# slbouknight/accelerated-ray-tracer

Hardware: AMD Instinct MI355X
Metric: Mrays/s, 1200x800 random scene @ 500 spp (frame ms in ms_per_step) (higher is better)
Workload: dtype f32

## Files before the change

accelerated-ray-tracer_amd/csrc/rt_abi.hip:

```cpp
#include <hip/hip_runtime.h>

#include <algorithm>
#include <cfloat>
#include <utility>
#include <cmath>
#include <functional>
#include <cstdio>
#include <cstring>
#include <string>
#include <vector>

#include "../../include/rt_abi.h"
#include "rt_call_buffers.h"
#include "rt_device.h"
#include "rt_frame_plan.h"
#include "rt_handoff_order.h"
#include "rt_refit_host.h"
#include "rt_scene_plan.h"

namespace {

struct device_info {
    bool ready = false;
    int num_cu = 256;
// ... 1553 lines not shown
    *count_out = (int64_t)count;
    const size_t n = count < (size_t)cap ? count : (size_t)cap;
    if (n == 0) return RT_OK;
    HIPCHK(hipMemcpy(entries, s->d_handoff, n * sizeof(unsigned long long), hipMemcpyDeviceToHost));
    HIPCHK(hipMemcpy(served, s->plan.tail_ordered ? s->d_handoff_ordered : s->d_handoff, n * sizeof(unsigned long long), hipMemcpyDeviceToHost));
    std::vector<rt_pixel_state> h_state(s->pixel_capacity);
    HIPCHK(hipMemcpy(h_state.data(), s->d_state, h_state.size() * sizeof(rt_pixel_state), hipMemcpyDeviceToHost));
    for (size_t i = 0; i < n; ++i) {
        const uint32_t pix = (uint32_t)entries[i];
        costs[i] = pix < h_state.size() ? h_state[pix].cost : 0u;
    }
    return RT_OK;
}

enum { ORDER_SEAM_SLACK = 3 };
rt_status rt_debug_order_handoff(const unsigned long long* entries, const uint32_t* costs, int64_t n, int32_t sample_begin, int32_t sample_end,
                                 int32_t tail_waves, unsigned long long* out, uint32_t* overrun_out) {
    if (!overrun_out) return invalid("rt_debug_order_handoff: null argument");
    if (n < 0 || n > (1ll << 24) || (n > 0 && (!entries || !costs || !out))) return invalid("rt_debug_order_handoff: n must be 0 .. 2^24 and the arrays non-null");
    if (sample_begin < 0 || sample_end < sample_begin) return invalid("rt_debug_order_handoff: bad sample range");
    if (tail_waves < 1 || tail_waves > (1 << 20)) return invalid("rt_debug_order_handoff: tail_waves must be 1 .. 2^20");
    for (int64_t i = 0; i < n; ++i)
        if ((int64_t)(uint32_t)entries[i] >= n) return invalid("rt_debug_order_handoff: an entry's pixel is not below n");
    RT_TRY(use_device(g_device));
    call_memory mem;
    rt_handoff_order_params hp;
    memset(&hp, 0, sizeof(hp));
    const size_t most = (size_t)RT_HANDOFF_ORDER_MAX_PER_WAVE * (size_t)tail_waves;
    hp.cap = (uint32_t)n; hp.min_items = (uint32_t)(RT_HANDOFF_ORDER_MIN_PER_WAVE * tail_waves); hp.max_items = (uint32_t)(most < (size_t)n ? most : (size_t)n);
    hp.cost_begin = sample_begin; hp.sample_end = sample_end;
    unsigned long long *d_queue = nullptr, *d_ordered = nullptr;
    rt_pixel_state* d_state = nullptr;
    unsigned int* d_pushed = nullptr;
    const size_t scratch_bytes = rt_handoff_order_scratch_words(hp.max_items) * sizeof(unsigned int);
    HIPCHK(mem.get((void**)&d_queue, (size_t)(n + ORDER_SEAM_SLACK) * sizeof(unsigned long long)));
    HIPCHK(mem.get((void**)&d_ordered, (size_t)(n + ORDER_SEAM_SLACK) * sizeof(unsigned long long)));
    HIPCHK(mem.get((void**)&d_state, (size_t)(n + 1) * sizeof(rt_pixel_state)));
    HIPCHK(mem.get((void**)&d_pushed, sizeof(unsigned int)));
    HIPCHK(mem.get((void**)&hp.scratch, scratch_bytes));
    std::vector<rt_pixel_state> h_state((size_t)n + 1);
    for (int64_t i = 0; i < n; ++i) h_state[(size_t)i].cost = costs[i];
    const unsigned int h_pushed = (unsigned int)n + ORDER_SEAM_SLACK;
    HIPCHK(hipMemset(d_queue, 0, (size_t)(n + ORDER_SEAM_SLACK) * sizeof(unsigned long long)));
    if (n > 0) HIPCHK(hipMemcpy(d_queue, entries, (size_t)n * sizeof(unsigned long long), hipMemcpyHostToDevice));
    HIPCHK(hipMemcpy(d_state, h_state.data(), h_state.size() * sizeof(rt_pixel_state), hipMemcpyHostToDevice));
    HIPCHK(hipMemset(d_ordered, 0xFF, (size_t)(n + ORDER_SEAM_SLACK) * sizeof(unsigned long long)));
    HIPCHK(hipMemcpy(d_pushed, &h_pushed, sizeof(h_pushed), hipMemcpyHostToDevice));
    HIPCHK(hipMemset(hp.scratch, 0, scratch_bytes));
    hp.queue = d_queue; hp.ordered = d_ordered; hp.state = d_state; hp.pushed = d_pushed;
    HIPCHK(rt_launch_handoff_order(hp, nullptr));
    HIPCHK(hipDeviceSynchronize());
    if (n > 0) HIPCHK(hipMemcpy(out, d_ordered, (size_t)n * sizeof(unsigned long long), hipMemcpyDeviceToHost));
    unsigned long long spare[ORDER_SEAM_SLACK];
    HIPCHK(hipMemcpy(spare, d_ordered + n, sizeof(spare), hipMemcpyDeviceToHost));
    *overrun_out = 0u;
    for (const unsigned long long w : spare) *overrun_out += w != ~0ull ? 1u : 0u;
    return RT_OK;
}

rt_status rt_debug_counters(rt_scene* s, unsigned long long* out16) {
    if (!s || !out16) return invalid("null argument");
    RT_TRY(use_device(s->device));
    HIPCHK(hipMemcpy(out16, s->d_ray_counter + 1, 16 * sizeof(unsigned long long), hipMemcpyDeviceToHost));
    return RT_OK;
}
rt_status rt_debug_stage_cycles(rt_scene* s, unsigned long long* out10) {
    if (!s || !out10) return invalid("null argument");
    RT_TRY(use_device(s->device));
    HIPCHK(hipMemcpy(out10, s->d_ray_counter + 17, 10 * sizeof(unsigned long long), hipMemcpyDeviceToHost));
    return RT_OK;
}
rt_status rt_debug_wave_ends(rt_scene* s, unsigned long long* out, int n) {
    if (!s || !out || n < 0 || n > 2 * RT_DIAG_BINS) return invalid("bad argument");
    RT_TRY(use_device(s->device));
    HIPCHK(hipMemcpy(out, s->d_ray_counter + RT_DIAG_HIST_SLOT, (size_t)n * sizeof(unsigned long long), hipMemcpyDeviceToHost));
    return RT_OK;
}
rt_status rt_debug_wave_last(rt_scene* s, unsigned long long* out, int n_waves) {
    if (!s || !out || n_waves < 0 || n_waves > RT_DIAG_MAX_WAVES) return invalid("bad argument");
    RT_TRY(use_device(s->device));
    HIPCHK(hipMemcpy(out, s->d_ray_counter + RT_DIAG_WAVE_SLOT, (size_t)2 * n_waves * sizeof(unsigned long long), hipMemcpyDeviceToHost));
    return RT_OK;
}

namespace {
enum { RANK_PARAM_WORDS = 20, RANK_INFO_WORDS = 13 };
static_assert(sizeof(rt_rank_info) == RANK_INFO_WORDS * 4, "rt_debug_rank / rt_debug_rank_info copy rt_rank_info as 13 words");
}

rt_status rt_debug_rank(const uint32_t* cost, const uint32_t* tile_cost, uint64_t rays, const uint32_t* params, uint32_t* tile_order,
                        uint32_t* cost_out, uint32_t* heavy_pixels, uint32_t* info13) {
    if (!cost || !tile_cost || !params || !tile_order || !cost_out || !heavy_pixels || !info13) return invalid("rt_debug_rank: null argument");
    rt_rank_params rp;
    memset(&rp, 0, sizeof(rp));
    const int32_t* ip = reinterpret_cast<const int32_t*>(params);
    rp.n_pixels = params[0]; rp.n_tiles = params[1]; rp.heavy_cap = params[2];
    rp.max_grid = params[3]; rp.waves_per_wg = params[4]; rp.normal_need = params[5];
    rp.sparse_stride = ip[6]; rp.semi_stride = ip[7]; rp.sparse_percent = ip[8]; rp.sparse_work_percent = ip[9];
    rp.tier_possible = ip[10]; rp.tier1_pixels = ip[11]; rp.tier1_depth = ip[12]; rp.tier_wgs_cap = ip[13];
    rp.tier_waves_per_main_wg = ip[14]; rp.nx = ip[15]; rp.smooth_percent = ip[16];
    memcpy(&rp.heavy_factor, params + 17, 4); memcpy(&rp.sparse_factor, params + 18, 4); memcpy(&rp.tier1_factor, params + 19, 4);
    if (rp.n_pixels < 1u || rp.n_pixels >= (1u << 31)) return invalid("rt_debug_rank: n_pixels must be 1 .. 2^31 - 1");
    if (rp.n_tiles < 1u || rp.n_tiles > rp.n_pixels) return invalid("rt_debug_rank: n_tiles must be 1 .. n_pixels");
    if (rp.heavy_cap < 1u || rp.heavy_cap > (1u << 24)) return invalid("rt_debug_rank: heavy_cap must be 1 .. 2^24");
    if (rp.max_grid > (1u << 20) || rp.normal_need > (1u << 20)) return invalid("rt_debug_rank: max_grid and normal_need must be at most 2^20");
    if (rp.waves_per_wg < 1u || rp.waves_per_wg > 16u) return invalid("rt_debug_rank: waves_per_wg must be 1 .. 16");
    if (rp.sparse_stride < 0 || rp.sparse_stride > 64 || rp.semi_stride < 0 || rp.semi_stride > 64) return invalid("rt_debug_rank: sparse_stride and semi_stride must be 0 .. 64");
    if (rp.sparse_percent < 0 || rp.sparse_percent > 100 || rp.sparse_work_percent < 0 || rp.sparse_work_percent > 100 || rp.smooth_percent < 0 || rp.smooth_percent > 100)
        return invalid("rt_debug_rank: sparse_percent, sparse_work_percent and smooth_percent must be 0 .. 100");
    if (rp.tier1_pixels < 0 || rp.tier1_depth < 0 || rp.tier1_depth > 65536 || rp.tier_wgs_cap < 0 || rp.tier_waves_per_main_wg < 0)
        return invalid("rt_debug_rank: tier1_pixels, tier1_depth (at most 65536), tier_wgs_cap and tier_waves_per_main_wg must not be negative");
    if (rp.nx < 1 || (uint32_t)rp.nx > rp.n_pixels) return invalid("rt_debug_rank: nx must be 1 .. n_pixels");
    float top = 0.f;
    for (const float fac : {rp.heavy_factor, rp.sparse_factor, rp.tier1_factor}) {
        if (!(fac >= 0.f) || !(fac <= 1000.f)) return invalid("rt_debug_rank: the three factors must be 0 .. 1000");
        top = fac > top ? fac : top;
    }
    if (!((double)rays / (double)rp.n_pixels * (double)top + 1.0 < 4294967296.0)) return invalid("rt_debug_rank: rays / n_pixels x the largest factor must stay below 2^32");
    RT_TRY(use_device(g_device));
    call_memory mem;
    unsigned int *d_tile_cost = nullptr, *d_tile_order = nullptr;
    unsigned long long* d_rays = nullptr;
    HIPCHK(mem.get((void**)&rp.state, (size_t)rp.n_pixels * sizeof(rt_pixel_state)));
    HIPCHK(mem.get((void**)&d_tile_cost, (size_t)rp.n_tiles * sizeof(unsigned int)));
    HIPCHK(mem.get((void**)&d_tile_order, (size_t)rp.n_tiles * sizeof(unsigned int)));
    HIPCHK(mem.get((void**)&d_rays, sizeof(unsigned long long)));
    HIPCHK(mem.get((void**)&rp.heavy_list, (size_t)rp.heavy_cap * sizeof(unsigned long long)));
    HIPCHK(mem.get((void**)&rp.heavy_pixels, (size_t)rp.heavy_cap * sizeof(unsigned int)));
    HIPCHK(mem.get((void**)&rp.info, sizeof(rt_rank_info)));
    rp.tile_cost = d_tile_cost; rp.tile_order = d_tile_order; rp.ray_counter = d_rays;
    std::vector<rt_pixel_state> h_state(rp.n_pixels);
    for (uint32_t i = 0; i < rp.n_pixels; ++i) h_state[i].cost = cost[i];
    const unsigned long long h_rays = rays;
    HIPCHK(hipMemcpy(rp.state, h_state.data(), (size_t)rp.n_pixels * sizeof(rt_pixel_state), hipMemcpyHostToDevice));
    HIPCHK(hipMemcpy(d_tile_cost, tile_cost, (size_t)rp.n_tiles * sizeof(unsigned int), hipMemcpyHostToDevice));
    HIPCHK(hipMemcpy(d_rays, &h_rays, sizeof(h_rays), hipMemcpyHostToDevice));
    HIPCHK(hipMemset(d_tile_order, 0xFF, (size_t)rp.n_tiles * sizeof(unsigned int)));
    HIPCHK(hipMemset(rp.heavy_list, 0xFF, (size_t)rp.heavy_cap * sizeof(unsigned long long)));
    HIPCHK(hipMemset(rp.heavy_pixels, 0xFF, (size_t)rp.heavy_cap * sizeof(unsigned int)));
    HIPCHK(hipMemset(rp.info, 0xFF, sizeof(rt_rank_info)));
    HIPCHK(rt_launch_rank(rp, nullptr));
    HIPCHK(hipDeviceSynchronize());
    HIPCHK(hipMemcpy(h_state.data(), rp.state, (size_t)rp.n_pixels * sizeof(rt_pixel_state), hipMemcpyDeviceToHost));
    for (uint32_t i = 0; i < rp.n_pixels; ++i) cost_out[i] = h_state[i].cost;
    HIPCHK(hipMemcpy(tile_order, d_tile_order, (size_t)rp.n_tiles * sizeof(unsigned int), hipMemcpyDeviceToHost));
    HIPCHK(hipMemcpy(heavy_pixels, rp.heavy_pixels, (size_t)rp.heavy_cap * sizeof(unsigned int), hipMemcpyDeviceToHost));
    HIPCHK(hipMemcpy(info13, rp.info, sizeof(rt_rank_info), hipMemcpyDeviceToHost));
    return RT_OK;
}

rt_status rt_debug_prior(const uint32_t* cal_cost, int32_t cal_nx, int32_t cal_ny, int32_t nx, int32_t ny, int32_t tile_rows, int32_t tile_first,
                         int32_t tile_stride, uint32_t* cost_out, uint32_t* tile_cost_out, uint64_t* total_out) {
    if (!cal_cost || !cost_out || !tile_cost_out || !total_out) return invalid("rt_debug_prior: null argument");
    if (cal_nx < 1 || cal_ny < 1 || (long long)cal_nx * cal_ny >= (1ll << 31)) return invalid("rt_debug_prior: bad calibration grid size");
    rt_frame_desc f;
    memset(&f, 0, sizeof(f));
    f.nx = nx; f.ny = ny; f.tile_rows = tile_rows; f.tile_first = tile_first; f.tile_stride = tile_stride;
    frame_geometry g;
    RT_TRY(check_frame("rt_debug_prior", &f, false, STATE_FRAME_TEXTS, g));
    if (g.local_rows == 0) return invalid("rt_debug_prior: the partition has no rows");
    RT_TRY(use_device(g_device));
    rt_prior_params pp;
    memset(&pp, 0, sizeof(pp));
    pp.cal_nx = cal_nx; pp.cal_ny = cal_ny; pp.nx = nx; pp.ny = ny; pp.local_rows = g.local_rows; pp.tiles_x = g.tiles_x;
    pp.tile_rows = tile_rows; pp.tile_first = tile_first; pp.tile_stride = tile_stride;
    const size_t n_pixels = g.n_pixels, n_tiles = (size_t)g.tiles_x * (size_t)g.tiles_y, n_cal = (size_t)cal_nx * (size_t)cal_ny;
// ... 702 lines not shown
```

accelerated-ray-tracer_amd/csrc/rt_device.h:

```cpp
#pragma once
#include <hip/hip_runtime.h>
#include <stdint.h>

#include "../../include/rt_abi.h"

#define RT_PERSISTENT_THREADS 512
#ifndef RT_LEAN_MIN_WAVES
#define RT_LEAN_MIN_WAVES 4
#endif
#ifndef RT_LEAN_MAX_THREADS
#define RT_LEAN_MAX_THREADS 512
#endif
#define RT_HEAVY_MAX_THREADS 768
#define RT_HEAVY_MIN_WAVES 3

#define RT_TIER_THREADS 256
enum { RT_DIAG_BINS = 192, RT_DIAG_T0_SLOT = 32, RT_DIAG_HIST_SLOT = 33, RT_DIAG_WAVE_SLOT = 33 + 2 * 192 + 7, RT_DIAG_MAX_WAVES = 8192,
       RT_COUNTER_BYTES = (33 + 2 * 192 + 7 + 2 * 8192) * 8 };
enum { RT_KERNEL_PIXEL = 0, RT_KERNEL_STAGED = 3 };

struct rt_pixel_state {
    uint32_t rng[6];
    float col[3];
    uint32_t cost;
};

struct rt_rank_info {
    uint32_t heavy_items;
    uint32_t heavy_threshold;
    uint32_t tier1_items;
    uint32_t tier2_items;
    int32_t tier1_wgs;
    int32_t main_skip_wgs;
    int32_t sparse_wgs;
    int32_t sparse_stride;
    int32_t semi_wgs;
    int32_t semi_stride;
    uint32_t threshold1;
    uint32_t threshold2;
    uint32_t collected;
};

struct rt_rank_params {
    rt_pixel_state* state;
    const unsigned int* tile_cost;
    unsigned int* tile_order;
    const unsigned long long* ray_counter;
    unsigned long long* heavy_list;
    unsigned int* heavy_pixels;
    rt_rank_info* info;
    uint32_t n_pixels, n_tiles, heavy_cap;
    uint32_t max_grid, waves_per_wg, normal_need;
    int32_t sparse_stride;
    int32_t semi_stride;
    int32_t sparse_percent;
    int32_t sparse_work_percent;
    int32_t tier_possible;
    int32_t tier1_pixels;
    int32_t tier1_depth;
    int32_t tier_wgs_cap;
    int32_t tier_waves_per_main_wg;
    int32_t nx, smooth_percent;
    float heavy_factor, sparse_factor, tier1_factor;
};

#define RT_NODE_SKIP(stored) (~(stored))
#define RT_WALK_PRIM_TABLE_BYTES(n_nodes) ((4 * (n_nodes) + 15) & ~15)

struct rt_scene_dev {
    const rt_node* nodes;
    const rt_node* nodes_ref;
    const rt_sphere* spheres;
    const rt_quad* quads;
    const rt_box* boxes;
    const rt_instance* instances;
    const rt_medium* media;
    const rt_material* materials;
    const rt_texture* textures;
    const uint8_t* images;
    int32_t n_nodes, n_nodes_ref, n_spheres, n_materials, n_textures;
    float bound[3];
    float bound_pad;
    const float4* leaf_lo;
    const float4* leaf_hi;
    const float* slot_ranges;
    int32_t n_leaves, n_slots;
    int32_t n_media_leaves;
    int32_t media_ord[2];
    rt_camera camera;
};

enum { RT_WC_DEAD = 64,
       RT_WC_PUSHED = 65,
       RT_WC_TAIL_HEAD = 66,
       RT_WORK_COUNTER_BYTES = 512 };
struct rt_frame_params {
    float* fb;
    unsigned long long* ray_counter;
    unsigned int* work_counter;
    unsigned int* pixel_cost;
    unsigned int* node_pass;
// ... 359 lines not shown
```

accelerated-ray-tracer_amd/csrc/rt_kernel_tier.h:

```cpp
#pragma once
#include "rt_device_funcs.h"
#include "rt_launch.h"

struct TierView {
    const float4* lo;
    const float4* hi;
    const float* ranges;
    int n_slots;
    int n_media;
    int med_ord0, med_ord1;
};

template <bool FEW>
DEV float wave_min_of(float v, bool have) {
    if (!FEW) {
        float r = have ? v : FLT_MAX;
#pragma unroll
        for (int off = 32; off > 0; off >>= 1) r = fminf(r, __shfl_xor(r, off, 64));
        return r;
    }
    unsigned long long m = __ballot(have);
    float r = FLT_MAX;
    while (m != 0ull) {
        const int l = __ffsll((long long)m) - 1;
        m &= m - 1ull;
        r = fminf(r, __int_as_float(__builtin_amdgcn_readlane(__float_as_int(v), l)));
    }
    return r;
}

template <bool SPHERES_ONLY>
DEV bool trace_wave(const TierView& tv, const SceneView& sc, const Ray& r, HitInfo& best) {
    const f3 inv = mk3(1.0f / r.d.x, 1.0f / r.d.y, 1.0f / r.d.z);
    const float tmin = 0.001f;
    const float a = dot(r.d, r.d);
    const int lane = (int)(threadIdx.x & 63u);
    const bool finite = inv_is_finite(inv);
    bool meets = false;
    if (finite && lane < tv.n_slots) {
        const float* q = tv.ranges + lane * 8;
        float t_enter, t_exit;
        slab_interval(make_float4(q[0], q[1], q[2], 0.f), make_float4(q[3], q[4], q[5], 0.f), r.o, inv, tmin, t_enter, t_exit);
        meets = !(t_exit <= t_enter);
    }
    unsigned long long slot_mask = __ballot(meets);
    float bt = FLT_MAX;
    int bord = -1;
    int32_t bleaf = -1, binst = -1;
    bool bincl = false, anomaly = false;
    float pre0 = FLT_MAX, pre1 = FLT_MAX;
    if (SPHERES_ONLY) {
        int np = 0;
        int32_t p0 = -1, p1 = -1;
        int o0 = 0, o1 = 0;
        float e0 = 0.f, e1 = 0.f;
        auto sphere_candidate = [&](int32_t prim, int ord, float t_enter) {
            float t;
            if (sphere_test_a(sc.spheres[RT_PRIM_INDEX(prim)], r, a, tmin, FLT_MAX, t)) {
                if (!(t > t_enter)) anomaly = true;
                if (t < bt || (t == bt && ord < bord)) { bt = t; bord = ord; bleaf = prim; }
            }
        };
        auto note = [&](bool pass, int32_t prim, int ord, float t_enter) {
            const bool overflow = pass && np >= 2;
            if (pass && np == 0) { p0 = prim; o0 = ord; e0 = t_enter; }
            if (pass && np == 1) { p1 = prim; o1 = ord; e1 = t_enter; }
            if (pass) ++np;
            if (__ballot(overflow) != 0ull) { if (overflow) sphere_candidate(prim, ord, t_enter); }
        };
        while (slot_mask != 0ull) {
            const int k0 = __ffsll((long long)slot_mask) - 1;
            slot_mask &= slot_mask - 1ull;
            const bool two = slot_mask != 0ull;
            const int k1 = two ? __ffsll((long long)slot_mask) - 1 : k0;
            if (two) slot_mask &= slot_mask - 1ull;
            const int ord0 = k0 * 64 + lane, ord1 = k1 * 64 + lane;
            const float4 lo0 = tv.lo[ord0], hi0 = tv.hi[ord0], lo1 = tv.lo[ord1], hi1 = tv.hi[ord1];
            float t_enter, t_exit;
            slab_interval(lo0, hi0, r.o, inv, tmin, t_enter, t_exit);
            note(__float_as_int(lo0.w) >= 0 && !(t_exit <= t_enter), __float_as_int(lo0.w), ord0, t_enter);
            if (two) {
                slab_interval(lo1, hi1, r.o, inv, tmin, t_enter, t_exit);
                note(__float_as_int(lo1.w) >= 0 && !(t_exit <= t_enter), __float_as_int(lo1.w), ord1, t_enter);
            }
        }
        if (__ballot(np >= 1) != 0ull) { if (np >= 1) sphere_candidate(p0, o0, e0); }
        if (__ballot(np >= 2) != 0ull) { if (np >= 2) sphere_candidate(p1, o1, e1); }
    } else {
    auto candidate = [&](int32_t prim, int32_t inst1, int ord8, float t_enter) {
        Ray q = r;
        if (inst1 != 0) q = to_object_space(sc.instances[inst1 - 1], r);
        float t;
        const bool is_quad = RT_PRIM_KIND(prim) == RT_PRIM_QUAD;
        const bool hit = is_quad ? quad_test(sc.quads[RT_PRIM_INDEX(prim)], q, tmin, FLT_MAX, t) : sphere_test(sc.spheres[RT_PRIM_INDEX(prim)], q, tmin, FLT_MAX, t);
        if (hit) {
            if (!(t > t_enter)) anomaly = true;
            const bool better = t < bt || (t == bt && (is_quad ? (!bincl || ord8 > bord) : (!bincl && ord8 < bord)));
            if (better) { bt = t; bord = ord8; bleaf = prim; binst = inst1 - 1; bincl = is_quad; }
            if ((ord8 >> 3) < tv.med_ord0) pre0 = fminf(pre0, t);
            if ((ord8 >> 3) < tv.med_ord1) pre1 = fminf(pre1, t);
        }
    };
    while (slot_mask != 0ull) {
        const int k = __ffsll((long long)slot_mask) - 1;
        slot_mask &= slot_mask - 1ull;
        const int ord = k * 64 + lane;
        const float4 lo4 = tv.lo[ord], hi4 = tv.hi[ord];
        const int32_t prim = __float_as_int(lo4.w), xw = __float_as_int(hi4.w);
        float t_enter, t_exit;
        slab_interval(lo4, hi4, r.o, inv, tmin, t_enter, t_exit);
        const bool pass = prim >= 0 && !(t_exit <= t_enter) && RT_PRIM_KIND(prim) != RT_PRIM_MEDIUM;
        const bool six = (xw & (1 << 30)) != 0;
        const unsigned long long m1 = __ballot(pass && !six), m6 = __ballot(pass && six);
        if (m1 != 0ull) { if (pass && !six) candidate(prim, xw & 0x3FFFFFFF, ord * 8, t_enter); }
        if (m6 != 0ull) {
            const int need = 6 * __popcll(m6);
            for (int base = 0; base < need; base += 64) {
                const int j = base + lane;
                const int T = j / 6, f = j - 6 * T;
                int lo_l = 0, hi_l = 63;
#pragma unroll
                for (int it = 0; it < 6; ++it) {
                    const int mid = (lo_l + hi_l) >> 1;
                    const bool enough = __popcll(m6 & ((2ull << mid) - 1ull)) > T;
                    hi_l = enough ? mid : hi_l;
                    lo_l = enough ? lo_l : mid + 1;
                }
                const int src = lo_l & 63;
                const int32_t p0 = __shfl(prim, src, 64), x0 = __shfl(xw, src, 64);
                const float te = __shfl(t_enter, src, 64);
                if (j < need) candidate(p0 + f, x0 & 0x3FFFFFFF, (k * 64 + src) * 8 + f, te);
            }
        }
    }
    }
    if (!finite || __ballot(anomaly) != 0ull) return trace<SPHERES_ONLY>(sc, r, best);
    float tm[2] = {FLT_MAX, FLT_MAX};
    bool hm[2] = {false, false};
    if (!SPHERES_ONLY) {
        for (int m = 0; m < tv.n_media; ++m) {
            const int ord = m == 0 ? tv.med_ord0 : tv.med_ord1;
            float limit = wave_min_of<false>(m == 0 ? pre0 : pre1, (m == 0 ? pre0 : pre1) < FLT_MAX);
            if (m == 1 && hm[0]) limit = fminf(limit, tm[0]);
            const float4 lo4 = tv.lo[ord], hi4 = tv.hi[ord];
            const int32_t prim = __builtin_amdgcn_readfirstlane(__float_as_int(lo4.w));
            float t_enter, t_exit;
            slab_interval(lo4, hi4, r.o, inv, tmin, t_enter, t_exit);
            if (!(fminf(t_exit, limit) <= t_enter)) {
                const rt_medium med = uniform_load(sc.media + RT_PRIM_INDEX(prim));
                float t;
                if (medium_test<true>(sc, med, r, tmin, limit, t)) { tm[m] = t; hm[m] = true; }
            }
        }
    }
    const float ts = wave_min_of<SPHERES_ONLY>(bt, bord >= 0);
    const float tmin_all = fminf(ts, fminf(tm[0], tm[1]));
    best.inst = -1;
    if (!(tmin_all < FLT_MAX)) { best.t = FLT_MAX; best.prim = -1; return false; }
    unsigned long long tie = __ballot(bord >= 0 && bt == tmin_all);
    int w_ord = -1, w_lane = -1;
    bool w_incl = false;
    while (tie != 0ull) {
        const int l = __ffsll((long long)tie) - 1;
        tie &= tie - 1ull;
        const int o = __builtin_amdgcn_readlane(bord, l);
        const bool ic = __builtin_amdgcn_readlane(bincl ? 1 : 0, l) != 0;
        const bool take = w_ord < 0 || (ic ? (!w_incl || o > w_ord) : (!w_incl && o < w_ord));
        if (take) { w_ord = o; w_lane = l; w_incl = ic; }
    }
    int w_medium = -1;
    if (!SPHERES_ONLY) {
        for (int m = 0; m < tv.n_media; ++m) {
            if (!hm[m] || tm[m] != tmin_all) continue;
            const int o = (m == 0 ? tv.med_ord0 : tv.med_ord1) * 8;
            if (w_ord < 0 || !w_incl || o > w_ord) { w_ord = o; w_incl = true; w_medium = m; w_lane = -1; }
        }
    }
    best.t = tmin_all;
    if (w_medium >= 0) {
        const float4 lo4 = tv.lo[SPHERES_ONLY ? w_ord : (w_ord >> 3)];
        best.prim = __builtin_amdgcn_readfirstlane(__float_as_int(lo4.w));
        return true;
    }
    best.prim = __builtin_amdgcn_readlane(bleaf, w_lane);
    best.inst = SPHERES_ONLY ? -1 : __builtin_amdgcn_readlane(binst, w_lane);
    return true;
}

template <bool SPHERES_ONLY, int TEX, bool NEED_UV, bool LDS_SCENE>
__global__ void __launch_bounds__(RT_TIER_THREADS, (SPHERES_ONLY && TEX < 2) ? 4 : 3) rt_tier_kernel(rt_scene_dev sd, rt_frame_params fp) {
    extern __shared__ __attribute__((aligned(16))) unsigned char lds[];
    const bool tail = (fp.tail_mode & 1) != 0;
    const rt_rank_info* q = fp.rank;
    const uint32_t n_items = tail ? (fp.work_counter[RT_WC_PUSHED] < fp.handoff_cap ? fp.work_counter[RT_WC_PUSHED] : fp.handoff_cap) : q->tier1_items;
    const int my_wgs = tail ? (int)((n_items + RT_TIER_THREADS / 64 - 1) / (RT_TIER_THREADS / 64)) : q->tier1_wgs;
    if ((int)blockIdx.x >= my_wgs) return;
    if (fp.tier_priority >= 3) __builtin_amdgcn_s_setprio(3);
    else if (fp.tier_priority == 2) __builtin_amdgcn_s_setprio(2);
    else if (fp.tier_priority == 1) __builtin_amdgcn_s_setprio(1);

    SceneView sc;
    sc.nodes = sd.nodes; sc.spheres = sd.spheres; sc.quads = sd.quads; sc.boxes = sd.boxes; sc.instances = sd.instances;
    sc.media = sd.media; sc.materials = sd.materials; sc.textures = sd.textures; sc.images = sd.images; sc.n_nodes = sd.n_nodes;
    TierView tv;
    {
        const int n_pad = sd.n_slots * 64;
        float4* dlo = reinterpret_cast<float4*>(lds);
        float4* dhi = dlo + n_pad;
        float4* dr = dhi + n_pad;
        for (int k = (int)threadIdx.x; k < n_pad; k += (int)blockDim.x) { dlo[k] = sd.leaf_lo[k]; dhi[k] = sd.leaf_hi[k]; }
        const float4* sr = reinterpret_cast<const float4*>(sd.slot_ranges);
        for (int k = (int)threadIdx.x; k < sd.n_slots * 2; k += (int)blockDim.x) dr[k] = sr[k];
        if (LDS_SCENE) {
            float4* dsph = dr + sd.n_slots * 2;
            const float4* s4 = reinterpret_cast<const float4*>(sd.spheres);
            for (int k = (int)threadIdx.x; k < sd.n_spheres * 2; k += (int)blockDim.x) dsph[k] = s4[k];
            sc.spheres = reinterpret_cast<const rt_sphere*>(dsph);
            float4* dmat = dsph + sd.n_spheres * 2;
            const float4* m4 = reinterpret_cast<const float4*>(sd.materials);
            for (int k = (int)threadIdx.x; k < sd.n_materials * 2; k += (int)blockDim.x) dmat[k] = m4[k];
            sc.materials = reinterpret_cast<const rt_material*>(dmat);
            float4* dtex = dmat + sd.n_materials * 2;
            const float4* t4 = reinterpret_cast<const float4*>(sd.textures);
            for (int k = (int)threadIdx.x; k < sd.n_textures * 4; k += (int)blockDim.x) dtex[k] = t4[k];
            sc.textures = reinterpret_cast<const rt_texture*>(dtex);
        }
        __syncthreads();
        tv.lo = dlo; tv.hi = dhi; tv.ranges = reinterpret_cast<const float*>(dr); tv.n_slots = sd.n_slots;
        tv.n_media = SPHERES_ONLY ? 0 : sd.n_media_leaves;
        tv.med_ord0 = tv.n_media > 0 ? sd.media_ord[0] : 0x7FFFFFFF;
        tv.med_ord1 = tv.n_media > 1 ? sd.media_ord[1] : 0x7FFFFFFF;
    }

    unsigned int rays = 0;
#ifdef RT_DIAG
    unsigned long long diag_trace = 0, diag_shade = 0, diag_rays = 0;
    const unsigned long long diag_t0 = __builtin_readcyclecounter();
#endif
    for (;;) {
        uint32_t idx = 0;
        if ((threadIdx.x & 63) == 0) idx = atomicAdd(fp.work_counter + (tail ? RT_WC_TAIL_HEAD : 2), 1u);
        idx = (uint32_t)__builtin_amdgcn_readfirstlane((int)idx);
        if (idx >= n_items) break;
        const unsigned long long item = tail ? fp.handoff_queue[idx] : (unsigned long long)fp.heavy_pixels[idx];
        const uint32_t pix = (uint32_t)item;
        const int first_sample = tail ? (int)(item >> 32) : fp.sample_begin;
        if (tail && (threadIdx.x & 63) == 0) {
            atomicAdd(fp.ray_counter + 28, 1ull); atomicAdd(fp.ray_counter + 29, (unsigned long long)(fp.sample_end - first_sample));
        }
        const int lrow = (int)(pix / (uint32_t)fp.nx), i = (int)(pix - (uint32_t)lrow * (uint32_t)fp.nx);
        const int j = local_to_global_row(fp, lrow);
        rt_xorwow pg;
        f3 pcol;
        uint32_t cost_before;
        {
            const rt_pixel_state st = tail ? fp.handoff_state[pix] : fp.state_in[pix];
            if (fp.fresh && !tail) {
                rt_xorwow_seed(pg, fp.seed_base + (uint64_t)(j * fp.nx + i));
                pcol = mk3(0, 0, 0);
                cost_before = st.cost & 0x80000000u;
            } else {
                pg.v0 = st.rng[0]; pg.v1 = st.rng[1]; pg.v2 = st.rng[2]; pg.v3 = st.rng[3]; pg.v4 = st.rng[4]; pg.d = st.rng[5];
                pcol = mk3(st.col[0], st.col[1], st.col[2]);
                cost_before = st.cost;
            }
        }
        unsigned int pixel_rays = 0;
        for (int sidx = first_sample; sidx < fp.sample_end; ++sidx) {
            const float u = ((float)i + rt_xorwow_uniform(pg)) / (float)fp.nx;
            const float v = ((float)j + rt_xorwow_uniform(pg)) / (float)fp.ny;
            Ray r = camera_get_ray(sd.camera, u, v, pg);
            f3 thr = mk3(1, 1, 1), rad = mk3(0, 0, 0);
            for (int depth = 0; depth < 50; ++depth) {
                HitInfo h;
                ++pixel_rays;
#ifdef RT_DIAG
                const unsigned long long dg0 = __builtin_readcyclecounter();
#endif
                const bool hit_something = trace_wave<SPHERES_ONLY>(tv, sc, r, h);
#ifdef RT_DIAG
                const unsigned long long dg1 = __builtin_readcyclecounter();
                diag_trace += dg1 - dg0; ++diag_rays;
#endif
                if (!hit_something) { rad = fma3(thr, miss_color(fp, r), rad); break; }
                const HitRec rec = resolve_hit<SPHERES_ONLY, NEED_UV>(sc, r, h);
                f3 emitted, attenuation;
                Ray scattered;
                const bool go_on = shade<TEX>(sc, r, rec, pg, emitted, attenuation, scattered);
#ifdef RT_DIAG
                diag_shade += __builtin_readcyclecounter() - dg1;
#endif
                rad = fma3(thr, emitted, rad);
                if (!go_on) break;
                thr = thr * attenuation;
                r = scattered;
            }
            pcol = pcol + rad;
        }
        if ((threadIdx.x & 63) == 0) {
            if (fp.state_out) {
                rt_pixel_state so;
                so.rng[0] = pg.v0; so.rng[1] = pg.v1; so.rng[2] = pg.v2; so.rng[3] = pg.v3; so.rng[4] = pg.v4; so.rng[5] = pg.d;
                so.col[0] = pcol.x; so.col[1] = pcol.y; so.col[2] = pcol.z;
                so.cost = cost_before + pixel_rays;
                fp.state_out[pix] = so;
                if (fp.tile_cost) atomicAdd(&fp.tile_cost[(lrow >> 3) * fp.tiles_x + (i >> 3)], pixel_rays);
            } else {
                store_sum(fp, i, lrow, pcol);
                if (fp.cost_out) fp.cost_out[pix] = (cost_before + pixel_rays) & 0x7FFFFFFFu;
            }
            rays += pixel_rays;
        }
    }
    if ((threadIdx.x & 63) == 0 && rays) atomicAdd(fp.ray_counter, (unsigned long long)rays);
#ifdef RT_DIAG
    if (threadIdx.x == 0 && diag_rays) {
        atomicAdd(fp.ray_counter + 15, diag_trace); atomicAdd(fp.ray_counter + 16, diag_rays);
        atomicAdd(fp.ray_counter + 25, diag_shade); atomicAdd(fp.ray_counter + 26, (unsigned long long)(__builtin_readcyclecounter() - diag_t0));
    }
#endif
}

template <bool SO, int TX, bool UV, bool LS>
static hipError_t rt_launch_tier_variant(const rt_scene_dev& sd, const rt_frame_params& fp, dim3 grid, size_t lds, hipStream_t st) {
    return rt_launch_kernel(rt_tier_kernel<SO, TX, UV, LS>, dim3(RT_TIER_THREADS), grid, lds, st, sd, fp);
}
template <bool SO, int TX, bool UV>
static hipError_t rt_launch_tier_one(const rt_scene_dev& sd, const rt_frame_params& fp, dim3 grid, size_t lds, hipStream_t st) {
    return fp.tier_lds_scene ? rt_launch_tier_variant<SO, TX, UV, true>(sd, fp, grid, lds, st) : rt_launch_tier_variant<SO, TX, UV, false>(sd, fp, grid, lds, st);
}
```

Baseline: 15620.

## Add lean wave-uniform sphere trace, resolve and shade path for tier kernel

```diff
diff --git a/accelerated-ray-tracer_amd/csrc/rt_abi.hip b/accelerated-ray-tracer_amd/csrc/rt_abi.hip
--- a/accelerated-ray-tracer_amd/csrc/rt_abi.hip
+++ b/accelerated-ray-tracer_amd/csrc/rt_abi.hip
@@ -1659,6 +1659,12 @@
     HIPCHK(hipMemcpy(out, s->d_ray_counter + RT_DIAG_WAVE_SLOT, (size_t)2 * n_waves * sizeof(unsigned long long), hipMemcpyDeviceToHost));
     return RT_OK;
 }
+rt_status rt_debug_tier_phases(rt_scene* s, unsigned long long* out, int n) {
+    if (!s || !out || n < 0 || n > 2 * RT_DIAG_TIER_WORDS) return invalid("bad argument");
+    RT_TRY(use_device(s->device));
+    HIPCHK(hipMemcpy(out, s->d_ray_counter + RT_DIAG_TIER_SLOT, (size_t)n * sizeof(unsigned long long), hipMemcpyDeviceToHost));
+    return RT_OK;
+}
 
 namespace {
 enum { RANK_PARAM_WORDS = 20, RANK_INFO_WORDS = 13 };
diff --git a/accelerated-ray-tracer_amd/csrc/rt_device.h b/accelerated-ray-tracer_amd/csrc/rt_device.h
--- a/accelerated-ray-tracer_amd/csrc/rt_device.h
+++ b/accelerated-ray-tracer_amd/csrc/rt_device.h
@@ -16,7 +16,8 @@
 
 #define RT_TIER_THREADS 256
 enum { RT_DIAG_BINS = 192, RT_DIAG_T0_SLOT = 32, RT_DIAG_HIST_SLOT = 33, RT_DIAG_WAVE_SLOT = 33 + 2 * 192 + 7, RT_DIAG_MAX_WAVES = 8192,
-       RT_COUNTER_BYTES = (33 + 2 * 192 + 7 + 2 * 8192) * 8 };
+       RT_DIAG_TIER_SLOT = 33 + 2 * 192 + 7 + 2 * 8192, RT_DIAG_TIER_WORDS = 64,
+       RT_COUNTER_BYTES = (33 + 2 * 192 + 7 + 2 * 8192 + 2 * 64) * 8 };
 enum { RT_KERNEL_PIXEL = 0, RT_KERNEL_STAGED = 3 };
 
 struct rt_pixel_state {
diff --git a/accelerated-ray-tracer_amd/csrc/rt_kernel_tier.h b/accelerated-ray-tracer_amd/csrc/rt_kernel_tier.h
--- a/accelerated-ray-tracer_amd/csrc/rt_kernel_tier.h
+++ b/accelerated-ray-tracer_amd/csrc/rt_kernel_tier.h
@@ -11,29 +11,38 @@
     int med_ord0, med_ord1;
 };
 
-template <bool FEW>
+#ifdef RT_DIAG
+struct TierDiag {
+    unsigned long long c[40];
+    unsigned long long last;
+    unsigned long long* record;
+    DEV void slots(int n) const { if (threadIdx.x == 0) atomicAdd(record + 16 + (n < 12 ? n : 12), 1ull); }
+    DEV void lap(int k) { const unsigned long long now = __builtin_readcyclecounter(); c[k] += now - last; last = now; }
+};
+#define RT_TIER_LAP(k) dg.lap(k)
+#define RT_TIER_COUNT(k, n) dg.c[k] += (unsigned long long)(n)
+#define RT_TIER_SLOTS(n) dg.slots(n)
+#define RT_TIER_DIAG_ARG , TierDiag& dg
+#define RT_TIER_DIAG_PASS , dg
+#else
+#define RT_TIER_LAP(k)
+#define RT_TIER_COUNT(k, n)
+#define RT_TIER_SLOTS(n)
+#define RT_TIER_DIAG_ARG
+#define RT_TIER_DIAG_PASS
+#endif
+
 DEV float wave_min_of(float v, bool have) {
-    if (!FEW) {
-        float r = have ? v : FLT_MAX;
+    float r = have ? v : FLT_MAX;
 #pragma unroll
-        for (int off = 32; off > 0; off >>= 1) r = fminf(r, __shfl_xor(r, off, 64));
-        return r;
-    }
-    unsigned long long m = __ballot(have);
-    float r = FLT_MAX;
-    while (m != 0ull) {
-        const int l = __ffsll((long long)m) - 1;
-        m &= m - 1ull;
-        r = fminf(r, __int_as_float(__builtin_amdgcn_readlane(__float_as_int(v), l)));
-    }
+    for (int off = 32; off > 0; off >>= 1) r = fminf(r, __shfl_xor(r, off, 64));
     return r;
 }
 
-template <bool SPHERES_ONLY>
 DEV bool trace_wave(const TierView& tv, const SceneView& sc, const Ray& r, HitInfo& best) {
     const f3 inv = mk3(1.0f / r.d.x, 1.0f / r.d.y, 1.0f / r.d.z);
     const float tmin = 0.001f;
-    const float a = dot(r.d, r.d);
+    [[maybe_unused]] const float a = dot(r.d, r.d);
     const int lane = (int)(threadIdx.x & 63u);
     const bool finite = inv_is_finite(inv);
     bool meets = false;
@@ -49,44 +58,6 @@
     int32_t bleaf = -1, binst = -1;
     bool bincl = false, anomaly = false;
     float pre0 = FLT_MAX, pre1 = FLT_MAX;
-    if (SPHERES_ONLY) {
-        int np = 0;
-        int32_t p0 = -1, p1 = -1;
-        int o0 = 0, o1 = 0;
-        float e0 = 0.f, e1 = 0.f;
-        auto sphere_candidate = [&](int32_t prim, int ord, float t_enter) {
-            float t;
-            if (sphere_test_a(sc.spheres[RT_PRIM_INDEX(prim)], r, a, tmin, FLT_MAX, t)) {
-                if (!(t > t_enter)) anomaly = true;
-                if (t < bt || (t == bt && ord < bord)) { bt = t; bord = ord; bleaf = prim; }
-            }
-        };
-        auto note = [&](bool pass, int32_t prim, int ord, float t_enter) {
-            const bool overflow = pass && np >= 2;
-            if (pass && np == 0) { p0 = prim; o0 = ord; e0 = t_enter; }
-            if (pass && np == 1) { p1 = prim; o1 = ord; e1 = t_enter; }
-            if (pass) ++np;
-            if (__ballot(overflow) != 0ull) { if (overflow) sphere_candidate(prim, ord, t_enter); }
-        };
-        while (slot_mask != 0ull) {
-            const int k0 = __ffsll((long long)slot_mask) - 1;
-            slot_mask &= slot_mask - 1ull;
-            const bool two = slot_mask != 0ull;
-            const int k1 = two ? __ffsll((long long)slot_mask) - 1 : k0;
-            if (two) slot_mask &= slot_mask - 1ull;
-            const int ord0 = k0 * 64 + lane, ord1 = k1 * 64 + lane;
-            const float4 lo0 = tv.lo[ord0], hi0 = tv.hi[ord0], lo1 = tv.lo[ord1], hi1 = tv.hi[ord1];
-            float t_enter, t_exit;
-            slab_interval(lo0, hi0, r.o, inv, tmin, t_enter, t_exit);
-            note(__float_as_int(lo0.w) >= 0 && !(t_exit <= t_enter), __float_as_int(lo0.w), ord0, t_enter);
-            if (two) {
-                slab_interval(lo1, hi1, r.o, inv, tmin, t_enter, t_exit);
-                note(__float_as_int(lo1.w) >= 0 && !(t_exit <= t_enter), __float_as_int(lo1.w), ord1, t_enter);
-            }
-        }
-        if (__ballot(np >= 1) != 0ull) { if (np >= 1) sphere_candidate(p0, o0, e0); }
-        if (__ballot(np >= 2) != 0ull) { if (np >= 2) sphere_candidate(p1, o1, e1); }
-    } else {
     auto candidate = [&](int32_t prim, int32_t inst1, int ord8, float t_enter) {
         Ray q = r;
         if (inst1 != 0) q = to_object_space(sc.instances[inst1 - 1], r);
@@ -133,14 +104,13 @@
             }
         }
     }
-    }
-    if (!finite || __ballot(anomaly) != 0ull) return trace<SPHERES_ONLY>(sc, r, best);
+    if (!finite || __ballot(anomaly) != 0ull) return trace<false>(sc, r, best);
     float tm[2] = {FLT_MAX, FLT_MAX};
     bool hm[2] = {false, false};
-    if (!SPHERES_ONLY) {
+    {
         for (int m = 0; m < tv.n_media; ++m) {
             const int ord = m == 0 ? tv.med_ord0 : tv.med_ord1;
-            float limit = wave_min_of<false>(m == 0 ? pre0 : pre1, (m == 0 ? pre0 : pre1) < FLT_MAX);
+            float limit = wave_min_of(m == 0 ? pre0 : pre1, (m == 0 ? pre0 : pre1) < FLT_MAX);
             if (m == 1 && hm[0]) limit = fminf(limit, tm[0]);
             const float4 lo4 = tv.lo[ord], hi4 = tv.hi[ord];
             const int32_t prim = __builtin_amdgcn_readfirstlane(__float_as_int(lo4.w));
@@ -153,7 +123,7 @@
             }
         }
     }
-    const float ts = wave_min_of<SPHERES_ONLY>(bt, bord >= 0);
+    const float ts = wave_min_of(bt, bord >= 0);
     const float tmin_all = fminf(ts, fminf(tm[0], tm[1]));
     best.inst = -1;
     if (!(tmin_all < FLT_MAX)) { best.t = FLT_MAX; best.prim = -1; return false; }
@@ -169,7 +139,7 @@
         if (take) { w_ord = o; w_lane = l; w_incl = ic; }
     }
     int w_medium = -1;
-    if (!SPHERES_ONLY) {
+    {
         for (int m = 0; m < tv.n_media; ++m) {
             if (!hm[m] || tm[m] != tmin_all) continue;
             const int o = (m == 0 ? tv.med_ord0 : tv.med_ord1) * 8;
@@ -178,13 +148,227 @@
     }
     best.t = tmin_all;
     if (w_medium >= 0) {
-        const float4 lo4 = tv.lo[SPHERES_ONLY ? w_ord : (w_ord >> 3)];
+        const float4 lo4 = tv.lo[w_ord >> 3];
         best.prim = __builtin_amdgcn_readfirstlane(__float_as_int(lo4.w));
         return true;
     }
     best.prim = __builtin_amdgcn_readlane(bleaf, w_lane);
-    best.inst = SPHERES_ONLY ? -1 : __builtin_amdgcn_readlane(binst, w_lane);
+    best.inst = __builtin_amdgcn_readlane(binst, w_lane);
     return true;
+}
+
+
+struct TierLane {
+    float4 rlo, rhi;
+    bool has_slot;
+    bool pick_y, pick_z;
+};
+DEV TierLane tier_lane(const TierView& tv) {
+    const int lane = (int)(threadIdx.x & 63u);
+    TierLane tl;
+    tl.has_slot = lane < tv.n_slots;
+    tl.rlo = make_float4(0.f, 0.f, 0.f, 0.f); tl.rhi = tl.rlo;
+    if (tl.has_slot) {
+        const float* q = tv.ranges + lane * 8;
+        tl.rlo = make_float4(q[0], q[1], q[2], 0.f); tl.rhi = make_float4(q[3], q[4], q[5], 0.f);
+    }
+    tl.pick_y = lane % 3 == 1; tl.pick_z = lane % 3 == 2;
+    return tl;
+}
+
+DEV float pick3(const TierLane& tl, f3 v) { return tl.pick_z ? v.z : (tl.pick_y ? v.y : v.x); }
+DEV f3 lanes012(float q) {
+    const int b = __float_as_int(q);
+    return mk3(__int_as_float(__builtin_amdgcn_readlane(b, 0)), __int_as_float(__builtin_amdgcn_readlane(b, 1)), __int_as_float(__builtin_amdgcn_readlane(b, 2)));
+}
+DEV f3 sdiv_wave(const TierLane& tl, f3 v, float t) { return lanes012(pick3(tl, v) / t); }
+DEV f3 rcp_wave(const TierLane& tl, f3 d) { return lanes012(1.0f / pick3(tl, d)); }
+DEV f3 unit_vector_wave(const TierLane& tl, f3 v) { return sdiv_wave(tl, v, length(v)); }
+
+DEV bool slab_pass(const float4 lo_skip, const float4 hi_prim, const f3 o, const f3 inv, float tmin, float& t_enter) {
+    const float x0 = (lo_skip.x - o.x) * inv.x, x1 = (hi_prim.x - o.x) * inv.x;
+    const float y0 = (lo_skip.y - o.y) * inv.y, y1 = (hi_prim.y - o.y) * inv.y;
+    const float z0 = (lo_skip.z - o.z) * inv.z, z1 = (hi_prim.z - o.z) * inv.z;
+    float lo = __builtin_amdgcn_fmed3f(tmin, x0, x1), hi = __builtin_amdgcn_fmed3f(FLT_MAX, x0, x1);
+    lo = __builtin_amdgcn_fmed3f(lo, y0, y1); hi = __builtin_amdgcn_fmed3f(hi, y0, y1);
+    lo = __builtin_amdgcn_fmed3f(lo, z0, z1); hi = __builtin_amdgcn_fmed3f(hi, z0, z1);
+    t_enter = lo;
+    return !(hi <= lo);
+}
+
+DEV bool trace_wave_lean(const TierView& tv, const TierLane& tl, const SceneView& sc, const Ray& r, HitInfo& best RT_TIER_DIAG_ARG) {
+    const f3 inv = rcp_wave(tl, r.d);
+    const float tmin = 0.001f;
+    const float a = dot(r.d, r.d);
+    const int lane = (int)(threadIdx.x & 63u);
+    const bool finite = inv_is_finite(inv);
+    bool meets = false;
+    if (finite && tl.has_slot) meets = slab_test_finite(tl.rlo, tl.rhi, r.o, inv, tmin, FLT_MAX);
+    unsigned long long slot_mask = __ballot(meets);
+    RT_TIER_LAP(1);
+    RT_TIER_SLOTS(__popcll(slot_mask));
+    float bt = FLT_MAX;
+    int bord = -1;
+    int32_t bleaf = -1;
+    bool anomaly = false;
+    int np = 0;
+    int32_t p0 = -1, p1 = -1;
+    int o0 = 0, o1 = 0;
+    float e0 = 0.f, e1 = 0.f;
+    auto sphere_candidate = [&](int32_t prim, int ord, float t_enter) {
+        float t;
+        if (sphere_test_a(sc.spheres[RT_PRIM_INDEX(prim)], r, a, tmin, FLT_MAX, t)) {
+            if (!(t > t_enter)) anomaly = true;
+            if (t < bt || (t == bt && ord < bord)) { bt = t; bord = ord; bleaf = prim; }
+        }
+    };
+    auto note = [&](bool pass, int32_t prim, int ord, float t_enter) -> bool {
+        const bool overflow = pass && np >= 2;
+        if (pass && np == 0) { p0 = prim; o0 = ord; e0 = t_enter; }
+        if (pass && np == 1) { p1 = prim; o1 = ord; e1 = t_enter; }
+        if (pass) ++np;
+        return overflow;
+    };
+    while (slot_mask != 0ull) {
+        RT_TIER_COUNT(3, 1);
+        const int k0 = __ffsll((long long)slot_mask) - 1;
+        slot_mask &= slot_mask - 1ull;
+        const bool has1 = slot_mask != 0ull;
+        const int k1 = has1 ? __ffsll((long long)slot_mask) - 1 : k0;
+        if (has1) slot_mask &= slot_mask - 1ull;
+        const bool has2 = slot_mask != 0ull;
+        const int k2 = has2 ? __ffsll((long long)slot_mask) - 1 : k1;
+        if (has2) slot_mask &= slot_mask - 1ull;
+        const bool has3 = slot_mask != 0ull;
+        const int k3 = has3 ? __ffsll((long long)slot_mask) - 1 : k2;
+        if (has3) slot_mask &= slot_mask - 1ull;
+        const int ord0 = k0 * 64 + lane, ord1 = k1 * 64 + lane, ord2 = k2 * 64 + lane, ord3 = k3 * 64 + lane;
+        const float4 lo0 = tv.lo[ord0], hi0 = tv.hi[ord0], lo1 = tv.lo[ord1], hi1 = tv.hi[ord1];
+        float4 lo2 = lo1, hi2 = hi1, lo3 = lo1, hi3 = hi1;
+        if (has2) { lo2 = tv.lo[ord2]; hi2 = tv.hi[ord2]; lo3 = tv.lo[ord3]; hi3 = tv.hi[ord3]; }
+        float te0, te1, te2 = 0.f, te3 = 0.f;
+        const bool in0 = slab_pass(lo0, hi0, r.o, inv, tmin, te0), in1 = slab_pass(lo1, hi1, r.o, inv, tmin, te1);
+        const bool pass0 = __float_as_int(lo0.w) >= 0 && in0;
+        const bool pass1 = has1 && __float_as_int(lo1.w) >= 0 && in1;
+        bool pass2 = false, pass3 = false;
+        if (has2) {
+            const bool in2 = slab_pass(lo2, hi2, r.o, inv, tmin, te2), in3 = slab_pass(lo3, hi3, r.o, inv, tmin, te3);
+            pass2 = __float_as_int(lo2.w) >= 0 && in2;
+            pass3 = has3 && __float_as_int(lo3.w) >= 0 && in3;
+        }
+        const bool ov0 = note(pass0, __float_as_int(lo0.w), ord0, te0);
+        const bool ov1 = note(pass1, __float_as_int(lo1.w), ord1, te1);
+        const bool ov2 = note(pass2, __float_as_int(lo2.w), ord2, te2);
+        const bool ov3 = note(pass3, __float_as_int(lo3.w), ord3, te3);
+        if (__ballot(ov0 || ov1 || ov2 || ov3) != 0ull) {
+            if (ov0) sphere_candidate(__float_as_int(lo0.w), ord0, te0);
+            if (ov1) sphere_candidate(__float_as_int(lo1.w), ord1, te1);
+            if (ov2) sphere_candidate(__float_as_int(lo2.w), ord2, te2);
+            if (ov3) sphere_candidate(__float_as_int(lo3.w), ord3, te3);
+        }
+    }
+    RT_TIER_LAP(2);
+    RT_TIER_COUNT(32, __popcll(__ballot(np == 1))); RT_TIER_COUNT(33, __popcll(__ballot(np == 2))); RT_TIER_COUNT(34, __popcll(__ballot(np >= 3)));
+    RT_TIER_COUNT(5, __ballot(np >= 2) != 0ull ? 1 : 0);
+    if (__ballot(np >= 1) != 0ull) { if (np >= 1) sphere_candidate(p0, o0, e0); }
+    if (__ballot(np >= 2) != 0ull) { if (np >= 2) sphere_candidate(p1, o1, e1); }
+    RT_TIER_LAP(4);
+    if (!finite || __ballot(anomaly) != 0ull) { RT_TIER_COUNT(11, 1); return trace<true>(sc, r, best); }
+    unsigned long long cand = __ballot(bord >= 0);
+    float w_t = FLT_MAX;
+    int w_ord = -1, w_lane = -1;
+    while (cand != 0ull) {
+        const int l = __ffsll((long long)cand) - 1;
+        cand &= cand - 1ull;
+        const float t = __int_as_float(__builtin_amdgcn_readlane(__float_as_int(bt), l));
+        const int o = __builtin_amdgcn_readlane(bord, l);
+        if (t < w_t || (t == w_t && o < w_ord)) { w_t = t; w_ord = o; w_lane = l; }
+    }
+    best.inst = -1;
+    if (w_lane < 0) { best.t = FLT_MAX; best.prim = -1; return false; }
+    best.t = w_t;
+    best.prim = __builtin_amdgcn_readlane(bleaf, w_lane);
+    return true;
+}
+
+template <bool NEED_UV>
+DEV HitRec resolve_sphere_wave(const TierLane& tl, const SceneView& sc, const Ray& r, const HitInfo& h) {
+    HitRec rec;
+    rec.u = 0.f; rec.v = 0.f;
+    const rt_sphere s = sc.spheres[RT_PRIM_INDEX(h.prim)];
+    const f3 cc = fma3(r.tm, ld3(s.vel), ld3(s.c0));
+    rec.p = ray_at(r, h.t);
+    rec.n = sdiv_wave(tl, rec.p - cc, s.radius);
+    if (NEED_UV && sc.materials[s.mat].pad != 0.0f) sphere_uv(rec.n, rec.u, rec.v);
+    rec.mat = s.mat;
+    return rec;
+}
+
+DEV bool refract_wave(const TierLane& tl, f3 v, f3 n, float ni_over_nt, f3& refracted) {
+    const f3 uv = unit_vector_wave(tl, v);
+    const float dt = dot(uv, n);
+    const float disc = fmaf(-(ni_over_nt * ni_over_nt), fmaf(-dt, dt, 1.0f), 1.0f);
+    if (disc > 0.0f) {
+        refracted = fma3(-sqrtf(disc), n, ni_over_nt * fma3(-dt, n, uv));
+        return true;
+    }
+    return false;
+}
+DEV f3 dielectric_direction_wave(const TierLane& tl, f3 d_in, f3 n, float ior, rt_xorwow& g) {
+    f3 outward_normal;
+    const f3 reflected = reflect(d_in, n);
+    float ni_over_nt, cosine, reflect_prob;
+    f3 refracted = mk3(0.f, 0.f, 0.f);
+    const float d_n = dot(d_in, n);
+    if (d_n > 0.0f) {
+        outward_normal = -n;
+        ni_over_nt = ior;
+        cosine = d_n / length(d_in);
+        cosine = sqrtf(fmaxf(0.0f, fmaf(-(ior * ior), fmaf(-cosine, cosine, 1.0f), 1.0f)));
+    } else {
+        outward_normal = n;
+        ni_over_nt = 1.0f / ior;
+        cosine = -d_n / length(d_in);
+    }
+    if (refract_wave(tl, d_in, outward_normal, ni_over_nt, refracted)) reflect_prob = schlick(cosine, ior);
+    else reflect_prob = 1.0f;
+    return (rt_xorwow_uniform(g) < reflect_prob) ? reflected : refracted;
+}
+template <int TEX>
+DEV bool shade_wave(const TierLane& tl, const SceneView& sc, const Ray& in, const HitRec& rec, rt_xorwow& g, f3& emitted, f3& attenuation, Ray& out) {
+    const rt_material m = sc.materials[rec.mat];
+    emitted = mk3(0.f, 0.f, 0.f);
+    out.o = rec.p;
+    out.tm = in.tm;
+    switch (m.kind) {
+    case RT_MAT_LAMBERTIAN: {
+        const f3 target = (rec.p + rec.n) + random_in_unit_sphere(g);
+        out.d = target - rec.p;
+        attenuation = (TEX > 0 && m.tex >= 0) ? texture_value<TEX>(sc, m.tex, rec.u, rec.v, rec.p) : ld3(m.albedo);
+        return true;
+    }
+    case RT_MAT_METAL: {
+        const f3 reflected = reflect(unit_vector_wave(tl, in.d), rec.n);
+        const f3 rs = random_in_unit_sphere(g);
+        out.d = fma3(m.fuzz, rs, reflected);
+        attenuation = ld3(m.albedo);
+        return dot(out.d, rec.n) > 0.0f;
+    }
+    case RT_MAT_DIELECTRIC: {
+        attenuation = mk3(1.0f, 1.0f, 1.0f);
+        out.d = dielectric_direction_wave(tl, in.d, rec.n, m.ior, g);
+        return true;
+    }
+    case RT_MAT_DIFFUSE_LIGHT: {
+        emitted = (TEX > 0 && m.tex >= 0) ? texture_value<TEX>(sc, m.tex, rec.u, rec.v, rec.p) : ld3(m.albedo);
+        return false;
+    }
+    default: {
+        out.d = random_in_unit_sphere(g);
+        attenuation = (TEX > 0 && m.tex >= 0) ? texture_value<TEX>(sc, m.tex, rec.u, rec.v, rec.p) : ld3(m.albedo);
+        return true;
+    }
+    }
 }
 
 template <bool SPHERES_ONLY, int TEX, bool NEED_UV, bool LDS_SCENE>
@@ -231,11 +415,17 @@
         tv.med_ord0 = tv.n_media > 0 ? sd.media_ord[0] : 0x7FFFFFFF;
         tv.med_ord1 = tv.n_media > 1 ? sd.media_ord[1] : 0x7FFFFFFF;
     }
+    TierLane tl;
+    if constexpr (SPHERES_ONLY) tl = tier_lane(tv);
 
     unsigned int rays = 0;
 #ifdef RT_DIAG
     unsigned long long diag_trace = 0, diag_shade = 0, diag_rays = 0;
     const unsigned long long diag_t0 = __builtin_readcyclecounter();
+    TierDiag dg;
+    for (int k = 0; k < 40; ++k) dg.c[k] = 0;
+    dg.last = diag_t0;
+    dg.record = fp.ray_counter + RT_DIAG_TIER_SLOT + (tail ? RT_DIAG_TIER_WORDS : 0);
 #endif
     for (;;) {
         uint32_t idx = 0;
@@ -267,26 +457,41 @@
         }
         unsigned int pixel_rays = 0;
         for (int sidx = first_sample; sidx < fp.sample_end; ++sidx) {
+            RT_TIER_LAP(12);
+            RT_TIER_COUNT(10, 1);
             const float u = ((float)i + rt_xorwow_uniform(pg)) / (float)fp.nx;
             const float v = ((float)j + rt_xorwow_uniform(pg)) / (float)fp.ny;
+            RT_TIER_LAP(13);
             Ray r = camera_get_ray(sd.camera, u, v, pg);
             f3 thr = mk3(1, 1, 1), rad = mk3(0, 0, 0);
+            RT_TIER_LAP(9);
             for (int depth = 0; depth < 50; ++depth) {
                 HitInfo h;
                 ++pixel_rays;
 #ifdef RT_DIAG
                 const unsigned long long dg0 = __builtin_readcyclecounter();
 #endif
-                const bool hit_something = trace_wave<SPHERES_ONLY>(tv, sc, r, h);
+                RT_TIER_LAP(12);
+                RT_TIER_COUNT(0, 1);
+                bool hit_something;
+                if constexpr (SPHERES_ONLY) hit_something = trace_wave_lean(tv, tl, sc, r, h RT_TIER_DIAG_PASS);
+                else hit_something = trace_wave(tv, sc, r, h);
+                RT_TIER_LAP(6);
 #ifdef RT_DIAG
                 const unsigned long long dg1 = __builtin_readcyclecounter();
                 diag_trace += dg1 - dg0; ++diag_rays;
 #endif
                 if (!hit_something) { rad = fma3(thr, miss_color(fp, r), rad); break; }
-                const HitRec rec = resolve_hit<SPHERES_ONLY, NEED_UV>(sc, r, h);
+                HitRec rec;
+                if constexpr (SPHERES_ONLY) rec = resolve_sphere_wave<NEED_UV>(tl, sc, r, h);
+                else rec = resolve_hit<false, NEED_UV>(sc, r, h);
+                RT_TIER_LAP(7);
                 f3 emitted, attenuation;
                 Ray scattered;
-                const bool go_on = shade<TEX>(sc, r, rec, pg, emitted, attenuation, scattered);
+                bool go_on;
+                if constexpr (SPHERES_ONLY) go_on = shade_wave<TEX>(tl, sc, r, rec, pg, emitted, attenuation, scattered);
+                else go_on = shade<TEX>(sc, r, rec, pg, emitted, attenuation, scattered);
+                RT_TIER_LAP(8);
 #ifdef RT_DIAG
                 diag_shade += __builtin_readcyclecounter() - dg1;
 #endif
@@ -317,6 +522,7 @@
     if (threadIdx.x == 0 && diag_rays) {
         atomicAdd(fp.ray_counter + 15, diag_trace); atomicAdd(fp.ray_counter + 16, diag_rays);
         atomicAdd(fp.ray_counter + 25, diag_shade); atomicAdd(fp.ray_counter + 26, (unsigned long long)(__builtin_readcyclecounter() - diag_t0));
+        for (int k = 0; k < 40; ++k) { if (k < 16 || k >= 32) atomicAdd(dg.record + k, dg.c[k]); }
     }
 #endif
 }
```

Result: no change. 15750, median of 6 (+0.8%).
